# lemerleau/RAFFT

Hardware: AMD Instinct MI355X
Metric: sequences/sec (whole node) on benchmark set, beam N=100; kcal/mol MAE vs CPU (higher is better)
Workload: dtype f32 FFT -> exact int counts, f64 scores, i32 dcal energies

## Files before the change

### rafft_amd/csrc/rafft_config.h

```cpp
#pragma once
#include <cstdio>
#include <cstdlib>
#include <cstring>

struct Config {
    double reserve_frac = 0.10;
    double est = 0.0;
    long linger_us = 600;
    long spin_us = 200, nap_us = 50;
    double big_wave_frac = 0.10;
    int cls1_p = 512;
    int c3_direct = 1;
    int c3_switch = -1;
    int direct_n = 1024;
    int force_fft = 0;
    int prod = 1;
    int no_memo = 0;
    int small_n4 = 16, small_n5 = 32;
    int small_wg = 4;
    int slab = 64;
    int fetch = 4, taper = 25;
    int mat_tile = 64;
    int rl_cap = -1;
    int wide_below = 600;
    int merge_below = -1;
    int merge2_below = -1;
    int split = -1;
    int serial = 0;
    int trace = 0;
    int spans = -1;
    int max_waves = 3;
    int merge_seqs = 16384;
    int trace_alloc = 0;
    int test_hard_fail = -1;
    int test_max_prod = 0;
    int test_ovf_at = -1;
    int seen_fixed = 0;
    int test_cand_limit = 0;
    int seen_bm_max = -1;
    int pad_ = 0;
};
static_assert(sizeof(Config) == 8 * 6 + 4 * 32, "Config: 8-byte fields first, an even number of ints - no padding (same_config compares bytes)");

inline Config read_config()
{
    Config c;
    auto I = [](const char *name, int &v) { if (const char *e = getenv(name)) v = atoi(e); };
    auto L = [](const char *name, long &v) { if (const char *e = getenv(name)) v = atol(e); };
    auto F = [](const char *name, double &v) { if (const char *e = getenv(name)) v = atof(e); };
    auto B = [](const char *name, int &v) { if (getenv(name)) v = 1; };
    I("RAFFT_CLS1_P", c.cls1_p); I("RAFFT_C3_DIRECT", c.c3_direct); I("RAFFT_C3_SWITCH", c.c3_switch); I("RAFFT_DIRECT_N", c.direct_n);
    I("RAFFT_FORCE_FFT", c.force_fft); I("RAFFT_PROD", c.prod); I("RAFFT_NO_MEMO", c.no_memo);
    if (const char *e = getenv("RAFFT_SMALL")) { int a = 16, b = 32; if (sscanf(e, "%d,%d", &a, &b) >= 1) { c.small_n4 = a; c.small_n5 = b; } }
    I("RAFFT_SMALL_WG", c.small_wg); I("RAFFT_SLAB", c.slab); I("RAFFT_FETCH", c.fetch); I("RAFFT_TAPER", c.taper);
    I("RAFFT_WIDE_BELOW", c.wide_below); I("RAFFT_MERGE_BELOW", c.merge_below); I("RAFFT_MERGE2_BELOW", c.merge2_below);
    F("RAFFT_RESERVE_FRAC", c.reserve_frac); I("RAFFT_SPLIT", c.split); I("RAFFT_SERIAL", c.serial);
    I("RAFFT_TRACE", c.trace); if (getenv("RAFFT_TRACE") && c.trace < 1) c.trace = 1;
    I("RAFFT_SPANS", c.spans);
    I("RAFFT_MAX_WAVES", c.max_waves); I("RAFFT_MERGE_SEQS", c.merge_seqs);
    L("RAFFT_LINGER_US", c.linger_us); L("RAFFT_SCHED_SPIN_US", c.spin_us); L("RAFFT_SCHED_NAP_US", c.nap_us); F("RAFFT_BIG_WAVE_FRAC", c.big_wave_frac);
    B("RAFFT_TRACE_ALLOC", c.trace_alloc);
#ifndef RAFFT_NO_TEST_HOOKS
    I("RAFFT_MAT_TILE", c.mat_tile); I("RAFFT_RL_CAP", c.rl_cap); F("RAFFT_EST", c.est); I("RAFFT_SEEN_FIXED", c.seen_fixed);
    I("RAFFT_TEST_CAND_LIMIT", c.test_cand_limit); I("RAFFT_TEST_HARD_FAIL", c.test_hard_fail); I("RAFFT_TEST_MAX_PROD", c.test_max_prod); I("RAFFT_TEST_OVF_AT", c.test_ovf_at);
    I("RAFFT_SEEN_BM_MAX", c.seen_bm_max);
#endif
    return c;
}
inline bool same_config(const Config &a, const Config &b) { return memcmp(&a, &b, sizeof(Config)) == 0; }
```

### rafft_amd/csrc/rafft_kernels.h

```cpp
#pragma once
#include "rafft_device.h"

struct alignas(16) Cand {
    int32_t ddcal;
    uint16_t mi, mj, nb, cut_hi;
    uint32_t cut_lo;
    uint64_t h1, h2;
    __host__ __device__ void set_cuts(int lo0, int hi0, int loo, int hio)
    {
        const unsigned long long v = (unsigned long long)lo0 | ((unsigned long long)hi0 << 12) | ((unsigned long long)loo << 24) | ((unsigned long long)hio << 36);
        cut_lo = (uint32_t)v; cut_hi = (uint16_t)(v >> 32);
    }
    __host__ __device__ void get_cuts(int &lo0, int &hi0, int &loo, int &hio) const
    {
        const unsigned long long v = (unsigned long long)cut_lo | ((unsigned long long)cut_hi << 32);
        lo0 = (int)(v & 4095); hi0 = (int)((v >> 12) & 4095); loo = (int)((v >> 24) & 4095); hio = (int)((v >> 36) & 4095);
    }
};
static_assert(sizeof(Cand) == 32, "Cand must be 32 bytes");

#define NSHARD 64
#ifndef SEEN0
#define SEEN0 8192
#endif
// ... 8 lines not shown
    uint64_t h1, h2;
    uint64_t sp, cursor, combo, total, prod;
    uint64_t c0h1, c0h2;
    uint64_t pad2[3];
};
static_assert(sizeof(StRec) == 128, "StRec is two cache lines");

struct alignas(64) NodeRec {
    int32_t seq, pdcal, n, ci, cj, nbr, ncand, L;
    uint64_t pos, br, cand, soff;
};
static_assert(sizeof(NodeRec) == 64, "NodeRec must be one cache line");

struct ProdEnt { uint32_t cnt; int32_t node; uint64_t off; };
struct alignas(16) MatRec { int32_t sid, sq, L, dcal, nprod, pad; uint64_t combo, prod, soff; };

struct Counters {
    unsigned int n_mat;
    unsigned int overflow;
    unsigned int n_done;
    unsigned int max_nprod;
    unsigned int pad0_[12];
    unsigned long long n_struct, pad1_[7];
    unsigned long long trec_n, tsid_top, pad2_[6];
    unsigned long long seen_top, pad3_[7];
    struct WorkCtr { unsigned int v; unsigned int pad[15]; } n_work[NCLS];
    unsigned long long n_expand, sum_n, sum_lags, n_children, sum_struct_len, n_alias, sum_nbr;
    unsigned long long cls_items[NCLS], cls_sum_n[NCLS], cls_sum_lags[NCLS];
    ShardCtr node[NSHARD], pos[NSHARD], br[NSHARD], sp[NSHARD], cand[NSHARD], node_prev[NSHARD], prod[NSHARD];
    ShardCtr nlist[NSHARD];
    ShardCtr wcur[NCLS][NSHARD];
    unsigned long long wdone[NCLS];
    unsigned long long wdone_pad[8 - NCLS];
    struct StatLine { unsigned long long items, n, lags, nbr, alias, children, struct_len, evals, guessed, kept_guessed, pad[6]; } xstat[NCLS][NSHARD];
};

enum { OVF_STRUCT = 1, OVF_NODE = 2, OVF_POS = 4, OVF_SP = 8, OVF_CAND = 16, OVF_SEEN = 32,
       OVF_TRAJ = 64, OVF_WORK = 128, OVF_PROD = 256, OVF_SORT = 512, OVF_BR = 1024, OVF_LOOPTAB = 2048, OVF_PRODLIST = 4096 };

struct DebugOut {
    int *n_ranked, *lag, *nb, *mi, *mj, *ddcal, *kept;
    double *corval, *score;
};

struct Dev {
    const EnergyTables *T;
    const float2 *tw;
    int S;
    const uint8_t *codes;
    const int *seq_off, *seq_len;
    int K, B, max_branch, min_hp, traj, memo, force_fft, rl_cap, mat_tile, merge_cls;
    double *big_keyv; size_t big_stride;
    int max_prod;
    int fetch_bulk, taper_pct;
    int direct_n;
    int sm_n4, sm_n5;
    int cand_slab;
    int cls1_P, cls1_br;
    int c3_switch;
    double min_nrj, gc, au, gu;
    int *beam, *beam_n, *done, *nsteps;
    int ch_cap;
    uint16_t *ch_parent; uint64_t *ch_combo; int *ch_dcal; uint64_t *ch_h;
    uint64_t *seen; uint64_t seen_cap_total;
    uint64_t *seen_off; uint32_t *seen_cap, *seen_cnt;
    uint32_t *seen_bm;
    uint32_t *seen_mode;
// ... 101 lines not shown
```

### rafft_amd/csrc/rafft_materialize.hip

```cpp
#pragma once


struct MatDesc {
    unsigned long long srcpos, srcbr, cidx;
    int pn, mi, mj, nb, n, nbr, ci, cj, lo0, hi0, loo, hio, a0, b0, ao, bo, flags, win;
    uint32_t newbr;
    int nnod, npos_in, npos_out, nbr_in, nbr_out;
};
__device__ inline MatDesc mat_describe(const Dev &d, int pn, unsigned long long cidx)
{
    MatDesc m;
    m.pn = pn;
    const Cand cd = d.cand[cidx];
    const uint4 *hp = (const uint4 *)&d.nd[pn];
    const uint4 hq0 = hp[0], hq1 = hp[1], hq2 = hp[2];
    m.n = (int)hq0.z; m.ci = (int)hq0.w; m.cj = (int)hq1.x; m.nbr = (int)hq1.y;
    m.srcpos = (unsigned long long)hq2.x | ((unsigned long long)hq2.y << 32); m.srcbr = (unsigned long long)hq2.z | ((unsigned long long)hq2.w << 32);
    m.cidx = cidx;
    m.mi = cd.mi; m.mj = cd.mj; m.nb = cd.nb;
    const uint16_t *pp = d.pos + m.srcpos;
    const int pm = d.pos_packed ? 0x0FFF : 0xFFFF;
    const uint32_t rao = pp[m.mi - m.nb + 1], rbo = pp[m.mj + m.nb - 1];
    m.a0 = pp[m.mi] & pm; m.b0 = pp[m.mj] & pm; m.ao = (int)rao & pm; m.bo = (int)rbo & pm;
    m.newbr = rao | (rbo << 16);
// ... 16 lines not shown
        uint32_t v[U];
#pragma unroll
        for (int u = 0; u < U; u++) {
            const int f = f0 + u * STR;
            v[u] = 0;
            if (f < tp) {
                int lo = 0, hi = 2 * kt - 1;
                while (lo < hi) { const int mid = (lo + hi + 1) >> 1; if (ps[mid] <= f) lo = mid; else hi = mid - 1; }
                const int kk = kb + (lo >> 1), off = f - ps[lo];
                const uint16_t *pp = d.pos + k_srcpos[kk];
                int src;
                if (!(lo & 1)) src = k_mi[kk] + 1 + off;
                else { const int left = k_mi[kk] - k_nb[kk] + 1; src = off < left ? off : k_mj[kk] + k_nb[kk] + (off - left); }
                v[u] = pp[src];
            }
        }
#pragma unroll
        for (int u = 0; u < U; u++) { const int f = f0 + u * STR; if (f < tp) d.pos[pdst + f] = (uint16_t)v[u]; }
    }
    for (int f0 = l; f0 < tbr; f0 += STR * U) {
        uint32_t v[U];
#pragma unroll
        for (int u = 0; u < U; u++) {
            const int f = f0 + u * STR;
            v[u] = 0;
            if (f < tbr) {
                int lo = 0, hi = 2 * kt - 1;
                while (lo < hi) { const int mid = (lo + hi + 1) >> 1; if (bs[mid] <= f) lo = mid; else hi = mid - 1; }
                const int kk = kb + (lo >> 1), off = f - bs[lo];
                const uint32_t *bb = d.br + k_srcbr[kk];
                if (!(lo & 1)) v[u] = bb[k_lo0[kk] + off];
                else {
                    const int loo = k_loo[kk];
                    v[u] = off < loo ? bb[off] : off == loo ? (uint32_t)k_newbr[kk] : bb[k_hio[kk] + (off - loo - 1)];
                }
            }
        }
#pragma unroll
        for (int u = 0; u < U; u++) { const int f = f0 + u * STR; if (f < tbr) d.br[bdst + f] = v[u]; }
    }
    for (int f0 = l; f0 < ts; f0 += STR * U) {
        uint32_t va[U], vb[U];
#pragma unroll
        for (int u = 0; u < U; u++) {
            const int f = f0 + u * STR;
            va[u] = 0; vb[u] = 0;
            if (f < ts) {
                int lo = 0, hi = kt - 1;
                while (lo < hi) { const int mid = (lo + hi + 1) >> 1; if (ns[mid] <= f) lo = mid; else hi = mid - 1; }
                const int t = f - ns[lo];
                const uint16_t *pp = d.pos + k_srcpos[kb + lo];
                va[u] = pp[k_mi[kb + lo] - t]; vb[u] = pp[k_mj[kb + lo] + t];
            }
        }
#pragma unroll
        for (int u = 0; u < U; u++) { const int f = f0 + u * STR; if (f < ts) d.sp[sdst + f] = (uint32_t)(va[u] & pmask) | ((uint32_t)(vb[u] & pmask) << 16); }
    }
}

#ifndef RAFFT_MAT_WAVES
#define RAFFT_MAT_WAVES 1
#endif
constexpr int MAT_NT = 64;
constexpr int MAT4_TL = 16;
constexpr int MAT4_TEAMS = 64 / MAT4_TL;
constexpr int MAT4_PROD = 64;

template <int TL>
__device__ __forceinline__ int team_incl_scan(int x, int tl)
{
    if constexpr (TL == 16) return row16_incl_scan(x);
    else {
        static_assert(TL == 64, "a team is one DPP row or the whole wavefront");
        for (int o = 1; o < 64; o <<= 1) { const int y = __shfl_up(x, o, 64); if (tl >= o) x += y; }
        return x;
    }
}
template <int TL>
__device__ __forceinline__ int team_sum(int x)
{
    if constexpr (TL == 16) return __shfl(row16_incl_scan(x), TL - 1, TL);
    else {
        for (int o = 32; o > 0; o >>= 1) x += __shfl_xor(x, o, 64);
        return x;
    }
}

template <int TL>
__device__ __forceinline__ void materialize_body(const Dev d, int n_mat, unsigned long long *prod_off, int *prod_node, int *prod_cnt,
                                                 int *sel, int cap)
{
    constexpr int TEAMS = 64 / TL;
    const int tid = threadIdx.x, team = tid / TL, tl = tid % TL;
    __shared__ unsigned long long k_srcpos[64], k_srcbr[64];
    __shared__ int k_mi[64], k_mj[64], k_nb[64], k_lo0[64], k_loo[64], k_hio[64], k_newbr[64];
    __shared__ int ps_[TEAMS][2 * TL + 1], bs_[TEAMS][2 * TL + 1], ns_[TEAMS][TL + 1];
    __shared__ unsigned long long sh64_[TEAMS][5];
    int *ps = ps_[team], *bs = bs_[team], *ns = ns_[team];
    const int tb = team * TL;
    const unsigned long long tmask = (~0ULL >> (64 - TL)) << tb;
    if (d.c->overflow) return;
    for (int mat_i0 = blockIdx.x * TEAMS; mat_i0 < n_mat; mat_i0 += gridDim.x * TEAMS) {
    const int mat_i = mat_i0 + team;
    const bool live = mat_i < n_mat;
    MatRec rec;
    rec.sid = 0; rec.sq = 0; rec.L = 0; rec.dcal = 0; rec.nprod = 0; rec.combo = 0; rec.prod = 0; rec.soff = 0;
    if (live) rec = d.mat[mat_i];
    const int sid = rec.sid, sq = rec.sq, L = rec.L, my_dcal = rec.dcal;
    const uint64_t soff = rec.soff;
    const int pmask = d.pos_packed ? 0x0FFF : 0xFFFF;
    int mprod = rec.nprod;
    if (mprod > cap) mprod = cap;
    {
        const ProdEnt *pl = d.prod + rec.prod;
        for (int k = tl; k < mprod; k += TL) { const ProdEnt pe = pl[k]; prod_node[k] = pe.node; prod_cnt[k] = (int)pe.cnt; prod_off[k] = pe.off; sel[k] = 0; }
    }
    wave_sync();
    if (tl == 0) {
        unsigned long long idx = rec.combo;
        for (int k = mprod - 1; k >= 0 && idx; k--) {
            const unsigned int c = (unsigned int)prod_cnt[k];
            if (idx < (1ULL << 24)) {
                const unsigned int v = (unsigned int)idx;
                unsigned int q = (unsigned int)((float)v * __frcp_rn((float)c));
                int r = (int)(v - q * c);
                if (r < 0) { q--; r += (int)c; } else if (r >= (int)c) { q++; r -= (int)c; }
                sel[k] = r; idx = q;
            } else { const unsigned long long q = idx / c; sel[k] = (int)(idx - q * c); idx = q; }
        }
    }
    wave_sync();

    const int TILE = d.mat_tile < TL ? d.mat_tile : TL;
    const bool one_tile = mprod <= TILE;
    const bool memo = d.memo != 0;
    MatDesc md;
    md.flags = 0; md.win = 0; md.nnod = 0; md.npos_in = md.npos_out = md.nbr_in = md.nbr_out = 0; md.nb = 0; md.cidx = 0;
    int tot_nodes = 0, tot_new = 0, tot_pos = 0, tot_br = 0, tot_sp = 0;
    for (int base = 0; base < mprod; base += TILE) {
        const int k = base + tl;
        int nnod = 0, nnew = 0, npos = 0, nbrr = 0, nsp = 0;
        if (k < mprod && tl < TILE) {
            const unsigned long long cidx = prod_off[k] + (unsigned long long)sel[k];
            unsigned long long old = 0;
            if (memo) old = atomicOr(&d.cslot[cidx], 0x8000000080000000ULL);
            md = mat_describe(d, prod_node[k], cidx);
            int win = md.flags;
            if (memo) win &= ((old >> 31) & 1ULL ? 0 : 1) | ((old >> 63) & 1ULL ? 0 : 2);
            md.win = win;
            if (!one_tile) sel[k] |= win << 28;
            nnod = md.nnod; nnew = (win & 1) + (win >> 1); nsp = md.nb;
            npos = ((win & 1) ? md.npos_in : 0) + ((win & 2) ? md.npos_out : 0);
            nbrr = ((win & 1) ? md.nbr_in : 0) + ((win & 2) ? md.nbr_out : 0);
        }
        nnod = team_sum<TL>(nnod); nnew = team_sum<TL>(nnew); npos = team_sum<TL>(npos); nbrr = team_sum<TL>(nbrr); nsp = team_sum<TL>(nsp);
        tot_nodes += nnod; tot_new += nnew; tot_pos += npos; tot_br += nbrr; tot_sp += nsp;
    }
    bool ok = live;
    if (tl < 5 && live) {
        const int shd = mat_i & (NSHARD - 1);
        unsigned long long *ctr = tl == 0 ? &d.c->node[shd].v : tl == 1 ? &d.c->pos[shd].v : tl == 2 ? &d.c->sp[shd].v : tl == 3 ? &d.c->br[shd].v : &d.c->nlist[shd].v;
        const unsigned long long want = tl == 0 ? (unsigned long long)tot_new : tl == 1 ? (unsigned long long)tot_pos
                                      : tl == 2 ? (unsigned long long)tot_sp : tl == 3 ? (unsigned long long)tot_br : (unsigned long long)tot_nodes;
        const unsigned long long cap = tl == 0 || tl == 4 ? d.nd_shard_cap : tl == 1 ? d.pos_shard_cap : tl == 2 ? d.sp_shard_cap : d.br_shard_cap;
        const unsigned long long b0 = want ? atomicAdd(ctr, want) : 0ULL;
        const bool bad = b0 + want > cap;
        if (bad) atomicOr(&d.c->overflow, tl == 0 || tl == 4 ? OVF_NODE : tl == 1 ? OVF_POS : tl == 2 ? OVF_SP : OVF_BR);
        const unsigned long long origin = tl == 0 || tl == 4 ? d.nd_base : tl == 1 ? d.pos_base : 0ULL;
        sh64_[team][tl] = origin + (unsigned long long)shd * cap + b0;
        ok = !bad;
    }
    ok = ((__ballot(!ok) & tmask) == 0ULL) && live;
    wave_sync();
    if (!ok) { if (tl == 0 && live) { d.st[sid].nnodes = 0; d.st[sid].node0 = 0; d.st[sid].sp = 0; d.st[sid].nsp = 0; } }
    const unsigned long long nbase = sh64_[team][0], pbase = sh64_[team][1], sbase = sh64_[team][2], bbase = sh64_[team][3], lbase = sh64_[team][4];

    int run_nodes = 0, run_new = 0, run_pos = 0, run_br = 0, run_sp = 0;
    const int mp2 = ok ? mprod : 0;
    for (int base = 0; base < mp2; base += TILE) {
        const int k = base + tl;
        const int kt = mp2 - base < TILE ? mp2 - base : TILE;
        if (!one_tile) {
            md.flags = 0; md.win = 0; md.nnod = 0; md.npos_in = md.npos_out = md.nbr_in = md.nbr_out = 0; md.nb = 0;
            if (k < mp2 && tl < TILE) { md = mat_describe(d, prod_node[k], prod_off[k] + (unsigned long long)(sel[k] & 0x0FFFFFFF)); md.win = (sel[k] >> 28) & 3; }
        }
        const bool act = k < mp2 && tl < TILE;
        const int cp_in = act && (md.win & 1) ? md.npos_in : 0, cp_out = act && (md.win & 2) ? md.npos_out : 0;
        const int cb_in = act && (md.win & 1) ? md.nbr_in : 0, cb_out = act && (md.win & 2) ? md.nbr_out : 0;
        int xn = act ? md.nnod : 0, xw = act ? (md.win & 1) + (md.win >> 1) : 0, xp = cp_in + cp_out, xb = cb_in + cb_out, xs = act ? md.nb : 0;
        const int vn = xn, vw = xw, vp = xp, vb = xb, vs = xs;
        xn = team_incl_scan<TL>(xn, tl); xw = team_incl_scan<TL>(xw, tl); xp = team_incl_scan<TL>(xp, tl); xb = team_incl_scan<TL>(xb, tl);
        xs = team_incl_scan<TL>(xs, tl);
        const int tn = __shfl(xn, TL - 1, TL), tw = __shfl(xw, TL - 1, TL), tp = __shfl(xp, TL - 1, TL), tbr = __shfl(xb, TL - 1, TL),
                  ts = __shfl(xs, TL - 1, TL);
        const int p0 = xp - vp, b0 = xb - vb;
        ps[2 * tl] = p0; ps[2 * tl + 1] = p0 + cp_in;
        bs[2 * tl] = b0; bs[2 * tl + 1] = b0 + cb_in;
        ns[tl] = xs - vs;
        if (tl == 0) { ps[2 * TL] = tp; bs[2 * TL] = tbr; ns[TL] = ts; }
        if (act) {
            k_srcpos[tid] = md.srcpos; k_srcbr[tid] = md.srcbr;
            k_mi[tid] = md.mi; k_mj[tid] = md.mj; k_nb[tid] = md.nb; k_lo0[tid] = md.lo0; k_loo[tid] = md.loo; k_hio[tid] = md.hio;
            k_newbr[tid] = (int)md.newbr;
            int nid = (int)(nbase + run_new + (xw - vw));
            unsigned long long le = lbase + run_nodes + (xn - vn);
            const unsigned long long poff = pbase + run_pos + p0, boff = bbase + run_br + b0;
            const int slot0 = (int)(2 * md.cidx);
            if (md.flags & 1) {
                if (md.win & 1) {
                    d.nd[nid].seq = sq; d.nd[nid].pdcal = my_dcal; d.nd[nid].pos = poff; d.nd[nid].n = md.npos_in;
                    d.nd[nid].L = L; d.nd[nid].soff = soff;
                    d.nd[nid].ci = md.a0; d.nd[nid].cj = md.b0; d.nd[nid].br = boff; d.nd[nid].nbr = md.nbr_in;
                    d.nd[nid].ncand = -1; d.nd[nid].cand = 0;
                    if (memo) { d.nd_slot[nid] = (uint32_t)slot0; ((uint32_t *)d.cslot)[slot0] = (uint32_t)(nid + 1) | 0x80000000u; }
                    d.nlist[le] = memo ? -(slot0 + 1) : nid;
                    nid++;
                } else d.nlist[le] = -(slot0 + 1);
                le++;
            }
            if (md.flags & 2) {
                if (md.win & 2) {
                    d.nd[nid].seq = sq; d.nd[nid].pdcal = my_dcal; d.nd[nid].pos = poff + cp_in; d.nd[nid].n = md.npos_out;
                    d.nd[nid].L = L; d.nd[nid].soff = soff;
                    d.nd[nid].ci = md.ci; d.nd[nid].cj = md.cj; d.nd[nid].br = boff + cb_in; d.nd[nid].nbr = md.nbr_out;
                    d.nd[nid].ncand = -1; d.nd[nid].cand = 0;
                    if (memo) { d.nd_slot[nid] = (uint32_t)(slot0 + 1); ((uint32_t *)d.cslot)[slot0 + 1] = (uint32_t)(nid + 1) | 0x80000000u; }
                    d.nlist[le] = memo ? -(slot0 + 2) : nid;
                } else d.nlist[le] = -(slot0 + 2);
            }
        }
        wave_sync();
        mat_copy_tile<TL, 4>(d, tl, tb, kt, ps, bs, ns, k_srcpos, k_srcbr, k_mi, k_mj, k_nb, k_lo0, k_loo, k_hio, k_newbr, tp, tbr, ts,
                             pbase + run_pos, bbase + run_br, sbase + run_sp, pmask);
        run_nodes += tn; run_new += tw; run_pos += tp; run_br += tbr; run_sp += ts;
        wave_sync();
    }
    if (ok && tl == 0) { d.st[sid].node0 = (int)lbase; d.st[sid].nnodes = tot_nodes; d.st[sid].sp = sbase; d.st[sid].nsp = tot_sp; }
    wave_sync();
    }
}

__global__ __launch_bounds__(MAT_NT, RAFFT_MAT_WAVES) void materialize_kernel(Dev d, int n_mat)
{
    extern __shared__ __align__(16) uint8_t mat_dyn[];
    unsigned long long *prod_off = (unsigned long long *)mat_dyn;
    int *prod_node = (int *)(prod_off + d.max_prod);
    int *prod_cnt = prod_node + d.max_prod;
    int *sel = prod_cnt + d.max_prod;
    materialize_body<MAT_NT>(d, n_mat, prod_off, prod_node, prod_cnt, sel, d.max_prod);
}

__global__ __launch_bounds__(64, RAFFT_MAT_WAVES) void materialize_team_kernel(Dev d, int n_mat)
{
    __shared__ unsigned long long prod_off_[MAT4_TEAMS][MAT4_PROD];
    __shared__ int prod_node_[MAT4_TEAMS][MAT4_PROD], prod_cnt_[MAT4_TEAMS][MAT4_PROD], sel_[MAT4_TEAMS][MAT4_PROD];
    const int team = threadIdx.x / MAT4_TL;
    materialize_body<MAT4_TL>(d, n_mat, prod_off_[team], prod_node_[team], prod_cnt_[team], sel_[team], MAT4_PROD);
}


struct NodeWords { uint4 q0, q1, q2; };
__device__ __forceinline__ NodeWords load_node_words(const Dev &d, int nid)
{
    const uint4 *hp = (const uint4 *)&d.nd[nid];
    NodeWords w;
    w.q0 = hp[0]; w.q1 = hp[1]; w.q2 = hp[2];
    pin(w.q0); pin(w.q1); pin(w.q2);
    return w;
}
__device__ inline bool same_loop(const Dev &d, const NodeWords &a, int b)
{
    const NodeWords o = load_node_words(d, b);
    if (a.q0.x != o.q0.x || a.q0.z != o.q0.z || a.q0.w != o.q0.w || a.q1.x != o.q1.x || a.q1.y != o.q1.y) return false;
    const uint32_t *x = d.br + ((unsigned long long)a.q2.z | ((unsigned long long)a.q2.w << 32));
    const uint32_t *y = d.br + ((unsigned long long)o.q2.z | ((unsigned long long)o.q2.w << 32));
    const int k = (int)a.q1.y;
    for (int i = 0; i < k; i += 4) {
        unsigned int xa[4], ya[4];
#pragma unroll
        for (int u = 0; u < 4; u++) { xa[u] = i + u < k ? x[i + u] : 0u; ya[u] = i + u < k ? y[i + u] : 0u; }
#pragma unroll
        for (int u = 0; u < 4; u++) { pin(xa[u]); pin(ya[u]); }
        if (xa[0] != ya[0] || xa[1] != ya[1] || xa[2] != ya[2] || xa[3] != ya[3]) return false;
    }
    return true;
}

#ifndef DEDUPE_NT
#define DEDUPE_NT 512
#endif
// ... 88 lines not shown
```

### rafft_amd/csrc/rafft_wave.h

```cpp
#pragma once

namespace {

hipEvent_t next_event(std::vector<hipEvent_t> &used)
{
    hipEvent_t e = nullptr;
    if (!g.ev_free.empty()) { e = g.ev_free.back(); g.ev_free.pop_back(); }
    else if (hipEventCreate(&e) != hipSuccess) return nullptr;
    used.push_back(e);
    return e;
}

struct Span { hipEvent_t a, b; int kind; };
static int g_span_level = 1;
static inline bool span_on(int kind) { return g_span_level >= 2 || (g_span_level == 1 && kind == 11); }
#define SPAN_REC(ev, st, kind) do { if (span_on(kind)) HIPCHK(hipEventRecord((ev), (st))); } while (0)

struct HostOut {
    std::vector<rafft_seq_result> seq;
    std::vector<std::vector<int>> step_size, step_off;
    std::vector<int> one_size, one_off;
    std::vector<const char *> db_ptr;
    std::vector<const int *> dcal_ptr;
    std::vector<std::shared_ptr<struct PinChunk>> chunks;
// ... 338 lines not shown
        }
        if (int rc = launch_expand_cls(cfg, d, cls, cf, grid, cs)) return rc;
        if (cls == 1) bt.stats.n_expand_launches++;
        SPAN_REC(sp.b, cs, sp.kind);
        spans.push_back(sp);
        if (!inline_) {
            HIPCHK(hipEventRecord(ws.ev_join[cls], cs));
            HIPCHK(hipStreamWaitEvent(st, ws.ev_join[cls], 0));
        }
    }
    SPAN_REC(wall.b, st, 4);
    spans.push_back(wall);
    {
        Span sp{next_event(), next_event(), 1};
        SPAN_REC(sp.a, st, sp.kind);
        if (n_active < wide_below) hipLaunchKernelGGL((beam_step_kernel<1024>), dim3((unsigned)S), dim3(1024), bs_lds[1], st, d, c.sort_cap, (int)bs_bm[1]);
        else hipLaunchKernelGGL((beam_step_kernel<256>), dim3((unsigned)S), dim3(256), bs_lds[0], st, d, c.sort_cap, (int)bs_bm[0]);
        HIPCHK(hipGetLastError());
        SPAN_REC(sp.b, st, sp.kind);
        spans.push_back(sp);
    }
    steps++;
    HIPCHK(hipMemcpyAsync(ws.hot, ws.counters.p, hot_len, hipMemcpyDeviceToHost, st));
    HIPCHK(hipEventRecord(ws.ev_hot, st));
    t_issued = std::chrono::steady_clock::now();
    return 0;
}

int Wave::issue_materialize(unsigned nm)
{
    hipStream_t st = ws.stream;
    Span sp{next_event(), next_event(), 2};
    SPAN_REC(sp.a, st, sp.kind);
    if (d.max_prod <= MAT4_PROD)
        hipLaunchKernelGGL(materialize_team_kernel, dim3((nm + MAT4_TEAMS - 1) / MAT4_TEAMS), dim3(64), 0, st, d, (int)nm);
    else hipLaunchKernelGGL(materialize_kernel, dim3(nm), dim3(MAT_NT), mat_lds, st, d, (int)nm);
    HIPCHK(hipGetLastError());
    const unsigned merge_below = cfg.merge_below >= 0 ? (unsigned)cfg.merge_below : 2u * (unsigned)g.n_cu;
    const unsigned merge2_below = cfg.merge2_below >= 0 ? (unsigned)cfg.merge2_below : 128u * (unsigned)g.n_cu;
    d.merge_cls = seam ? 0 : nm < merge_below ? merge_target : nm < merge2_below ? 2 : 0;
    merged_now = d.merge_cls;
    const unsigned dd_grid = std::min<unsigned>((unsigned)g.n_cu * (1024u / DEDUPE_NT), (unsigned)std::min<unsigned long long>(0x7fffffffULL, (unsigned long long)nm * 4ULL / DEDUPE_NT + 2ULL));
    hipLaunchKernelGGL(dedupe_kernel, dim3(dd_grid), dim3(DEDUPE_NT), 0, st, d);
    HIPCHK(hipGetLastError());
    SPAN_REC(sp.b, st, sp.kind);
    spans.push_back(sp);
    return 0;
}

int Wave::after_beam()
{
    HostTimer acc_{ms_after};
    hipStream_t st = ws.stream;
    if (draining) return finish_done();
    const size_t hot_len = offsetof(Counters, node);
    memcpy(&hc, ws.hot, hot_len);
    if (hc.overflow) { ovf = hc.overflow; return finish(); }
    if (cfg.test_ovf_at >= 0 && depth == 0 && steps == cfg.test_ovf_at) { ovf = OVF_STRUCT; return finish(); }
    if (hc.n_mat == 0) return finish();
    n_active = (unsigned)S - hc.n_done;
    last_mat = hc.n_mat;
    const bool harvest_now = !p.traj && !seam && !harvested && S >= 256 && (size_t)hc.trec_n * 10 >= S * 7;
    const size_t harvest_n = (size_t)hc.trec_n;
    if (int rc = issue_materialize(hc.n_mat)) return rc;
    if (cfg.trace >= 2) {
        Counters h2;
        HIPCHK(hipMemcpyAsync(&h2, ws.counters.p, hot_len, hipMemcpyDeviceToHost, st));
        HIPCHK(hipStreamSynchronize(st));
        fprintf(stderr, "[rafft] step %d: n_mat %u -> work %u %u %u %u | small %u %u\n", steps, hc.n_mat, h2.n_work[0].v, h2.n_work[1].v, h2.n_work[2].v, h2.n_work[3].v, h2.n_work[4].v, h2.n_work[5].v);
// ... 126 lines not shown
            const double sh = hc.n_expand ? (double)hc.cls_items[c] / (double)hc.n_expand : 0.0;
            const int64_t v = 3 * (int64_t)hc.cls_sum_n[c] + 16 * (int64_t)hc.cls_sum_lags[c] + (int64_t)(sh * 3.0 * (double)(hc.sum_struct_len + sumL));
            if (c == 2) bt.stats.alg_bytes_expand_c2 += v;
            else if (c == 3 || c == 0) bt.stats.alg_bytes_expand_c3 += v;
            else if (c >= NGEN) bt.stats.alg_bytes_expand_small += v;
        }
        bt.stats.alg_bytes_beam += 2 * (int64_t)hc.sum_struct_len + 8 * (int64_t)(hc.n_struct - S);
        bt.stats.alg_bytes_expand_all += ex;
        bt.stats.alg_bytes += ex + 2 * (int64_t)hc.sum_struct_len + 8 * (int64_t)(hc.n_struct - S);
    }


    tail.stats = since(tail.t0);
    if (int rc = emit_rows(harvested, (size_t)hc.trec_n - harvested, false, &tail.gather)) return rc;
    tail.gather += tail.stats;
    if (harvested) {
        HIPCHK(hipEventRecord(ws.ev_copy, ws.copy_stream));
        HIPCHK(hipStreamWaitEvent(st, ws.ev_copy, 0));
    }
    HIPCHK(hipEventRecord(ws.ev_hot, st));
    finished = false; draining = true;
    return 0;
}

int Wave::finish_done_body()
{
    finished = true;
    const double tl_copy = since(tail.t0);
    const long long tot_bytes = last_rows_bytes;
    if (cfg.trace) {
        auto mx = [&](const ShardCtr *sc) { unsigned long long m = 0, t = 0; for (int i = 0; i < NSHARD; i++) { m = std::max(m, sc[i].v); t += sc[i].v; } return std::make_pair(m, t); };
        auto nd = mx(hc.node), po = mx(hc.pos), br = mx(hc.br), spr = mx(hc.sp), ca = mx(hc.cand), pr = mx(hc.prod), nl = mx(hc.nlist);
        fprintf(stderr, "[rafft] max productive regions per structure: %u (limit %d)\n", hc.max_nprod, d.max_prod);
        fprintf(stderr, "[rafft] arenas used/cap (max shard | total): st %llu/%zu  nd %llu/%llu|%llu  pos %llu/%llu|%llu  br %llu/%llu|%llu  sp %llu/%llu|%llu  cand %llu/%llu|%llu  prod %llu/%llu|%llu  nlist %llu/%llu|%llu  seen %llu/%zu  est %.1f\n",
                hc.n_struct, c.st, nd.first, (unsigned long long)d.nd_shard_cap, nd.second, po.first, (unsigned long long)d.pos_shard_cap, po.second,
                br.first, (unsigned long long)d.br_shard_cap, br.second, spr.first, (unsigned long long)d.sp_shard_cap, spr.second,
                ca.first, (unsigned long long)d.cand_shard_cap, ca.second, pr.first, (unsigned long long)d.prod_shard_cap, pr.second, nl.first, (unsigned long long)d.nd_shard_cap, nl.second, hc.seen_top, c.seen, est);
    }
    if (cfg.trace >= 2) {
        std::vector<uint32_t> cnt(S), cap(S);
        HIPCHK(hipMemcpy(cnt.data(), d.seen_cnt, S * 4, hipMemcpyDeviceToHost));
        HIPCHK(hipMemcpy(cap.data(), d.seen_cap, S * 4, hipMemcpyDeviceToHost));
        const int edges[] = {0, 80, 100, 130, 200, 300, 500, 1000, 2000, 1 << 30};
        for (int e = 0; e + 1 < (int)(sizeof(edges) / sizeof(edges[0])); e++) {
            unsigned long long n = 0, sum = 0, mxc = 0, grown = 0, slots = 0;
            for (size_t i = 0; i < S; i++) if (len[i] > edges[e] && len[i] <= edges[e + 1]) { n++; sum += cnt[i]; mxc = std::max<unsigned long long>(mxc, cnt[i]); grown += cap[i] > seen_cap0[i] ? 1 : 0; slots += cap[i]; }
            if (n) fprintf(stderr, "[rafft] seen sets, %d < L <= %d: %llu sequences, mean %llu entries, max %llu, %llu grew, %llu slots at the end\n", edges[e], edges[e + 1], n, sum / n, mxc, grown, slots);
        }
    }
    if (cfg.trace) fprintf(stderr, "[rafft] host time inside issue_step %.3f ms, inside after_beam (incl. nested issue_step and this tail) %.3f ms\n", ms_issue, ms_after);
    if (cfg.trace) fprintf(stderr, "[rafft] wave S=%zu setup %.2f ms, loop %.2f ms (%d steps), tail %.2f ms (counters %.3f, records+gather %.3f, rows out %.3f incl. %.1f MB D2H)\n",
                                       S, ms_setup, tail.ms_loop, steps, since(tail.t0), tail.stats, tail.gather - tail.stats, tl_copy - tail.gather, (double)tot_bytes / 1e6);
    return result = 0;
}

int run_seam(Batch &bt, const std::vector<SeqIn> &one, const SeamIn &sm)
{
    Wave w(g.ws[0], {std::shared_ptr<Batch>(&bt, [](Batch *) {})}, one, 4.0, &sm);
    if (int rc = w.setup()) return rc;
    Workspace &W = g.ws[0];
    {
        std::vector<uint16_t> packed(sm.pos);
        if (w.d.pos_packed) {
            for (auto &v : packed) v = (uint16_t)(v | (kBaseCode[(unsigned char)one[0].s[v]] << 12));
        }
        HIPCHK(hipMemcpy(W.pos.p, packed.data(), packed.size() * 2, hipMemcpyHostToDevice));
// ... 27 lines not shown
```

Before: 550,900.

## Compute combo digits per lane in team materialize and drop LDS product lists

The team materialize kernel no longer stages the product lists (node, count, offset) in shared memory. Each lane keeps its own product entry in registers and works out its combo digit with a saturating suffix-product scan across the team, which replaces the serial digit loop on lane 0. The kernel becomes a template over team size, with an optional 8-lane team chosen by a new config knob, and the one-tile path reuses the descriptor from the first pass instead of calling mat_describe again. It also adds per-shard counters for materialized structures and multi-tile cases, printed under trace. These counters cost an extra atomic per block, and the scan adds 64-bit multiplies and divides per lane.

```diff
diff --git a/rafft_amd/csrc/rafft_config.h b/rafft_amd/csrc/rafft_config.h
--- a/rafft_amd/csrc/rafft_config.h
+++ b/rafft_amd/csrc/rafft_config.h
@@ -38,7 +38,7 @@
     int seen_fixed = 0;
     int test_cand_limit = 0;
     int seen_bm_max = -1;
-    int pad_ = 0;
+    int mat_team = 16;
 };
 static_assert(sizeof(Config) == 8 * 6 + 4 * 32, "Config: 8-byte fields first, an even number of ints - no padding (same_config compares bytes)");
 
@@ -61,7 +61,7 @@
     L("RAFFT_LINGER_US", c.linger_us); L("RAFFT_SCHED_SPIN_US", c.spin_us); L("RAFFT_SCHED_NAP_US", c.nap_us); F("RAFFT_BIG_WAVE_FRAC", c.big_wave_frac);
     B("RAFFT_TRACE_ALLOC", c.trace_alloc);
 #ifndef RAFFT_NO_TEST_HOOKS
-    I("RAFFT_MAT_TILE", c.mat_tile); I("RAFFT_RL_CAP", c.rl_cap); F("RAFFT_EST", c.est); I("RAFFT_SEEN_FIXED", c.seen_fixed);
+    I("RAFFT_MAT_TILE", c.mat_tile); I("RAFFT_MAT_TEAM", c.mat_team); I("RAFFT_RL_CAP", c.rl_cap); F("RAFFT_EST", c.est); I("RAFFT_SEEN_FIXED", c.seen_fixed);
     I("RAFFT_TEST_CAND_LIMIT", c.test_cand_limit); I("RAFFT_TEST_HARD_FAIL", c.test_hard_fail); I("RAFFT_TEST_MAX_PROD", c.test_max_prod); I("RAFFT_TEST_OVF_AT", c.test_ovf_at);
     I("RAFFT_SEEN_BM_MAX", c.seen_bm_max);
 #endif
diff --git a/rafft_amd/csrc/rafft_kernels.h b/rafft_amd/csrc/rafft_kernels.h
--- a/rafft_amd/csrc/rafft_kernels.h
+++ b/rafft_amd/csrc/rafft_kernels.h
@@ -64,7 +64,7 @@
     ShardCtr wcur[NCLS][NSHARD];
     unsigned long long wdone[NCLS];
     unsigned long long wdone_pad[8 - NCLS];
-    struct StatLine { unsigned long long items, n, lags, nbr, alias, children, struct_len, evals, guessed, kept_guessed, pad[6]; } xstat[NCLS][NSHARD];
+    struct StatLine { unsigned long long items, n, lags, nbr, alias, children, struct_len, evals, guessed, kept_guessed, mat, mat_tiles, pad[4]; } xstat[NCLS][NSHARD];
 };
 
 enum { OVF_STRUCT = 1, OVF_NODE = 2, OVF_POS = 4, OVF_SP = 8, OVF_CAND = 16, OVF_SEEN = 32,
diff --git a/rafft_amd/csrc/rafft_materialize.hip b/rafft_amd/csrc/rafft_materialize.hip
--- a/rafft_amd/csrc/rafft_materialize.hip
+++ b/rafft_amd/csrc/rafft_materialize.hip
@@ -72,7 +72,8 @@
                 if (!(lo & 1)) v[u] = bb[k_lo0[kk] + off];
                 else {
                     const int loo = k_loo[kk];
-                    v[u] = off < loo ? bb[off] : off == loo ? (uint32_t)k_newbr[kk] : bb[k_hio[kk] + (off - loo - 1)];
+                    v[u] = (uint32_t)k_newbr[kk];
+                    if (off != loo) v[u] = bb[off < loo ? off : k_hio[kk] + (off - loo - 1)];
                 }
             }
         }
@@ -102,46 +103,93 @@
 #define RAFFT_MAT_WAVES 1
 #endif
 constexpr int MAT_NT = 64;
-constexpr int MAT4_TL = 16;
-constexpr int MAT4_TEAMS = 64 / MAT4_TL;
 constexpr int MAT4_PROD = 64;
 
 template <int TL>
 __device__ __forceinline__ int team_incl_scan(int x, int tl)
 {
     if constexpr (TL == 16) return row16_incl_scan(x);
-    else {
-        static_assert(TL == 64, "a team is one DPP row or the whole wavefront");
+    else if constexpr (TL == 8) {
+        const int y1 = __builtin_amdgcn_update_dpp(0, x, 0x111, 0xF, 0xF, true);
+        x += tl >= 1 ? y1 : 0;
+        const int y2 = __builtin_amdgcn_update_dpp(0, x, 0x112, 0xF, 0xF, true);
+        x += tl >= 2 ? y2 : 0;
+        x += __builtin_amdgcn_update_dpp(0, x, 0x114, 0xF, 0xA, true);
+        return x;
+    } else {
+        static_assert(TL == 64, "a team is half a DPP row, one row or the whole wavefront");
         for (int o = 1; o < 64; o <<= 1) { const int y = __shfl_up(x, o, 64); if (tl >= o) x += y; }
         return x;
     }
 }
 template <int TL>
-__device__ __forceinline__ int team_sum(int x)
-{
-    if constexpr (TL == 16) return __shfl(row16_incl_scan(x), TL - 1, TL);
+__device__ __forceinline__ int team_sum(int x, int tl)
+{
+    if constexpr (TL < 64) return __shfl(team_incl_scan<TL>(x, tl), TL - 1, TL);
     else {
         for (int o = 32; o > 0; o >>= 1) x += __shfl_xor(x, o, 64);
         return x;
     }
 }
 
+__device__ __forceinline__ unsigned long long combo_divmod(unsigned long long idx, unsigned int c, unsigned int &rem)
+{
+    if (idx < (1ULL << 24)) {
+        const unsigned int v = (unsigned int)idx;
+        unsigned int q = (unsigned int)((float)v * __frcp_rn((float)c));
+        int r = (int)(v - q * c);
+        if (r < 0) { q--; r += (int)c; } else if (r >= (int)c) { q++; r -= (int)c; }
+        rem = (unsigned int)r;
+        return q;
+    }
+    const unsigned long long q = idx / c;
+    rem = (unsigned int)(idx - q * c);
+    return q;
+}
+__device__ __forceinline__ void combo_digits_serial(unsigned long long idx, const int *cnt, int *sel, int mprod)
+{
+    for (int k = mprod - 1; k >= 0; k--) {
+        unsigned int r = 0;
+        if (idx) idx = combo_divmod(idx, (unsigned int)cnt[k], r);
+        sel[k] = (int)r;
+    }
+}
 template <int TL>
+__device__ __forceinline__ int combo_digit_lanes(unsigned long long idx, unsigned int cnt, int tl)
+{
+    const unsigned long long sat = idx + 1;
+    unsigned long long s = cnt < sat ? cnt : sat;
+#pragma unroll
+    for (int o = 1; o < TL; o <<= 1) {
+        const unsigned long long y = __shfl_down(s, o, TL);
+        if (tl + o < TL) { const unsigned long long lo = s * y; s = (__umul64hi(s, y) || lo > sat) ? sat : lo; }
+    }
+    s = __shfl_down(s, 1, TL);
+    if (tl == TL - 1) s = 1;
+    if (s > idx) return 0;
+    unsigned int r;
+    const unsigned long long q = s < (1ULL << 24) && idx < (1ULL << 24)
+        ? (unsigned long long)combo_divmod(idx, (unsigned int)s, r) : idx / s;
+    combo_divmod(q, cnt, r);
+    return (int)r;
+}
+
+template <int TL, bool LISTS>
 __device__ __forceinline__ void materialize_body(const Dev d, int n_mat, unsigned long long *prod_off, int *prod_node, int *prod_cnt,
                                                  int *sel, int cap)
 {
     constexpr int TEAMS = 64 / TL;
+    static_assert(TL >= 5, "five lanes of a team allocate from the five arenas");
     const int tid = threadIdx.x, team = tid / TL, tl = tid % TL;
     __shared__ unsigned long long k_srcpos[64], k_srcbr[64];
     __shared__ int k_mi[64], k_mj[64], k_nb[64], k_lo0[64], k_loo[64], k_hio[64], k_newbr[64];
     __shared__ int ps_[TEAMS][2 * TL + 1], bs_[TEAMS][2 * TL + 1], ns_[TEAMS][TL + 1];
     __shared__ unsigned long long sh64_[TEAMS][5];
-    int *ps = ps_[team], *bs = bs_[team], *ns = ns_[team];
     const int tb = team * TL;
-    const unsigned long long tmask = (~0ULL >> (64 - TL)) << tb;
     if (d.c->overflow) return;
-    for (int mat_i0 = blockIdx.x * TEAMS; mat_i0 < n_mat; mat_i0 += gridDim.x * TEAMS) {
-    const int mat_i = mat_i0 + team;
+    unsigned int st_mat = 0, st_tiles = 0;
+    {
+    const int mat_i = blockIdx.x * TEAMS + team;
     const bool live = mat_i < n_mat;
     MatRec rec;
     rec.sid = 0; rec.sq = 0; rec.L = 0; rec.dcal = 0; rec.nprod = 0; rec.combo = 0; rec.prod = 0; rec.soff = 0;
@@ -151,28 +199,36 @@
     const int pmask = d.pos_packed ? 0x0FFF : 0xFFFF;
     int mprod = rec.nprod;
     if (mprod > cap) mprod = cap;
-    {
-        const ProdEnt *pl = d.prod + rec.prod;
-        for (int k = tl; k < mprod; k += TL) { const ProdEnt pe = pl[k]; prod_node[k] = pe.node; prod_cnt[k] = (int)pe.cnt; prod_off[k] = pe.off; sel[k] = 0; }
-    }
-    wave_sync();
-    if (tl == 0) {
-        unsigned long long idx = rec.combo;
-        for (int k = mprod - 1; k >= 0 && idx; k--) {
-            const unsigned int c = (unsigned int)prod_cnt[k];
-            if (idx < (1ULL << 24)) {
-                const unsigned int v = (unsigned int)idx;
-                unsigned int q = (unsigned int)((float)v * __frcp_rn((float)c));
-                int r = (int)(v - q * c);
-                if (r < 0) { q--; r += (int)c; } else if (r >= (int)c) { q++; r -= (int)c; }
-                sel[k] = r; idx = q;
-            } else { const unsigned long long q = idx / c; sel[k] = (int)(idx - q * c); idx = q; }
-        }
-    }
-    wave_sync();
-
     const int TILE = d.mat_tile < TL ? d.mat_tile : TL;
     const bool one_tile = mprod <= TILE;
+    if (tl == 0 && live) { st_mat++; st_tiles += one_tile ? 0 : 1; }
+    const ProdEnt *pl = d.prod + rec.prod;
+    int my_node = 0, my_sel = 0;
+    unsigned long long my_off = 0;
+    if constexpr (LISTS) {
+        for (int k = tl; k < mprod; k += TL) { const ProdEnt pe = pl[k]; prod_node[k] = pe.node; prod_cnt[k] = (int)pe.cnt; prod_off[k] = pe.off; }
+        wave_sync();
+        if (tl == 0) combo_digits_serial(rec.combo, prod_cnt, sel, mprod);
+        wave_sync();
+    } else {
+        unsigned int cnt = 1;
+        if (one_tile && tl < mprod) { const ProdEnt pe = pl[tl]; my_node = pe.node; my_off = pe.off; cnt = pe.cnt; }
+        my_sel = combo_digit_lanes<TL>(rec.combo, cnt, tl);
+        if (!one_tile) for (int k = tl; k < mprod; k += TL) sel[k] = (int)pl[k].cnt;
+        wave_sync();
+        if (!one_tile && tl == 0) combo_digits_serial(rec.combo, sel, sel, mprod);
+        wave_sync();
+    }
+    auto entry = [&](int k, int &node) -> unsigned long long {
+        if constexpr (LISTS) { node = prod_node[k]; return prod_off[k] + (unsigned long long)(sel[k] & 0x0FFFFFFF); }
+        else {
+            if (one_tile) { node = my_node; return my_off + (unsigned long long)my_sel; }
+            const ProdEnt pe = pl[k];
+            node = pe.node;
+            return pe.off + (unsigned long long)(sel[k] & 0x0FFFFFFF);
+        }
+    };
+
     const bool memo = d.memo != 0;
     MatDesc md;
     md.flags = 0; md.win = 0; md.nnod = 0; md.npos_in = md.npos_out = md.nbr_in = md.nbr_out = 0; md.nb = 0; md.cidx = 0;
@@ -181,10 +237,11 @@
         const int k = base + tl;
         int nnod = 0, nnew = 0, npos = 0, nbrr = 0, nsp = 0;
         if (k < mprod && tl < TILE) {
-            const unsigned long long cidx = prod_off[k] + (unsigned long long)sel[k];
+            int node;
+            const unsigned long long cidx = entry(k, node);
             unsigned long long old = 0;
             if (memo) old = atomicOr(&d.cslot[cidx], 0x8000000080000000ULL);
-            md = mat_describe(d, prod_node[k], cidx);
+            md = mat_describe(d, node, cidx);
             int win = md.flags;
             if (memo) win &= ((old >> 31) & 1ULL ? 0 : 1) | ((old >> 63) & 1ULL ? 0 : 2);
             md.win = win;
@@ -193,7 +250,7 @@
             npos = ((win & 1) ? md.npos_in : 0) + ((win & 2) ? md.npos_out : 0);
             nbrr = ((win & 1) ? md.nbr_in : 0) + ((win & 2) ? md.nbr_out : 0);
         }
-        nnod = team_sum<TL>(nnod); nnew = team_sum<TL>(nnew); npos = team_sum<TL>(npos); nbrr = team_sum<TL>(nbrr); nsp = team_sum<TL>(nsp);
+        nnod = team_sum<TL>(nnod, tl); nnew = team_sum<TL>(nnew, tl); npos = team_sum<TL>(npos, tl); nbrr = team_sum<TL>(nbrr, tl); nsp = team_sum<TL>(nsp, tl);
         tot_nodes += nnod; tot_new += nnew; tot_pos += npos; tot_br += nbrr; tot_sp += nsp;
     }
     bool ok = live;
@@ -210,24 +267,24 @@
         sh64_[team][tl] = origin + (unsigned long long)shd * cap + b0;
         ok = !bad;
     }
-    ok = ((__ballot(!ok) & tmask) == 0ULL) && live;
+    ok = ((__ballot(!ok) & ((~0ULL >> (64 - TL)) << tb)) == 0ULL) && live;
     wave_sync();
-    if (!ok) { if (tl == 0 && live) { d.st[sid].nnodes = 0; d.st[sid].node0 = 0; d.st[sid].sp = 0; d.st[sid].nsp = 0; } }
-    const unsigned long long nbase = sh64_[team][0], pbase = sh64_[team][1], sbase = sh64_[team][2], bbase = sh64_[team][3], lbase = sh64_[team][4];
+    if (tl == 0 && live) {
+        if (ok) { d.st[sid].node0 = (int)sh64_[team][4]; d.st[sid].nnodes = tot_nodes; d.st[sid].sp = sh64_[team][2]; d.st[sid].nsp = tot_sp; }
+        else { d.st[sid].nnodes = 0; d.st[sid].node0 = 0; d.st[sid].sp = 0; d.st[sid].nsp = 0; }
+    }
 
     int run_nodes = 0, run_new = 0, run_pos = 0, run_br = 0, run_sp = 0;
     const int mp2 = ok ? mprod : 0;
-    for (int base = 0; base < mp2; base += TILE) {
+    auto tile2 = [&](const MatDesc &m, int base) __attribute__((always_inline)) {
+        int *ps = ps_[team], *bs = bs_[team], *ns = ns_[team];
+        const unsigned long long *ab = sh64_[team];
         const int k = base + tl;
         const int kt = mp2 - base < TILE ? mp2 - base : TILE;
-        if (!one_tile) {
-            md.flags = 0; md.win = 0; md.nnod = 0; md.npos_in = md.npos_out = md.nbr_in = md.nbr_out = 0; md.nb = 0;
-            if (k < mp2 && tl < TILE) { md = mat_describe(d, prod_node[k], prod_off[k] + (unsigned long long)(sel[k] & 0x0FFFFFFF)); md.win = (sel[k] >> 28) & 3; }
-        }
         const bool act = k < mp2 && tl < TILE;
-        const int cp_in = act && (md.win & 1) ? md.npos_in : 0, cp_out = act && (md.win & 2) ? md.npos_out : 0;
-        const int cb_in = act && (md.win & 1) ? md.nbr_in : 0, cb_out = act && (md.win & 2) ? md.nbr_out : 0;
-        int xn = act ? md.nnod : 0, xw = act ? (md.win & 1) + (md.win >> 1) : 0, xp = cp_in + cp_out, xb = cb_in + cb_out, xs = act ? md.nb : 0;
+        const int cp_in = act && (m.win & 1) ? m.npos_in : 0, cp_out = act && (m.win & 2) ? m.npos_out : 0;
+        const int cb_in = act && (m.win & 1) ? m.nbr_in : 0, cb_out = act && (m.win & 2) ? m.nbr_out : 0;
+        int xn = act ? m.nnod : 0, xw = act ? (m.win & 1) + (m.win >> 1) : 0, xp = cp_in + cp_out, xb = cb_in + cb_out, xs = act ? m.nb : 0;
         const int vn = xn, vw = xw, vp = xp, vb = xb, vs = xs;
         xn = team_incl_scan<TL>(xn, tl); xw = team_incl_scan<TL>(xw, tl); xp = team_incl_scan<TL>(xp, tl); xb = team_incl_scan<TL>(xb, tl);
         xs = team_incl_scan<TL>(xs, tl);
@@ -239,18 +296,18 @@
         ns[tl] = xs - vs;
         if (tl == 0) { ps[2 * TL] = tp; bs[2 * TL] = tbr; ns[TL] = ts; }
         if (act) {
-            k_srcpos[tid] = md.srcpos; k_srcbr[tid] = md.srcbr;
-            k_mi[tid] = md.mi; k_mj[tid] = md.mj; k_nb[tid] = md.nb; k_lo0[tid] = md.lo0; k_loo[tid] = md.loo; k_hio[tid] = md.hio;
-            k_newbr[tid] = (int)md.newbr;
-            int nid = (int)(nbase + run_new + (xw - vw));
-            unsigned long long le = lbase + run_nodes + (xn - vn);
-            const unsigned long long poff = pbase + run_pos + p0, boff = bbase + run_br + b0;
-            const int slot0 = (int)(2 * md.cidx);
-            if (md.flags & 1) {
-                if (md.win & 1) {
-                    d.nd[nid].seq = sq; d.nd[nid].pdcal = my_dcal; d.nd[nid].pos = poff; d.nd[nid].n = md.npos_in;
+            k_srcpos[tid] = m.srcpos; k_srcbr[tid] = m.srcbr;
+            k_mi[tid] = m.mi; k_mj[tid] = m.mj; k_nb[tid] = m.nb; k_lo0[tid] = m.lo0; k_loo[tid] = m.loo; k_hio[tid] = m.hio;
+            k_newbr[tid] = (int)m.newbr;
+            int nid = (int)(ab[0] + run_new + (xw - vw));
+            unsigned long long le = ab[4] + run_nodes + (xn - vn);
+            const unsigned long long poff = ab[1] + run_pos + p0, boff = ab[3] + run_br + b0;
+            const int slot0 = (int)(2 * m.cidx);
+            if (m.flags & 1) {
+                if (m.win & 1) {
+                    d.nd[nid].seq = sq; d.nd[nid].pdcal = my_dcal; d.nd[nid].pos = poff; d.nd[nid].n = m.npos_in;
                     d.nd[nid].L = L; d.nd[nid].soff = soff;
-                    d.nd[nid].ci = md.a0; d.nd[nid].cj = md.b0; d.nd[nid].br = boff; d.nd[nid].nbr = md.nbr_in;
+                    d.nd[nid].ci = m.a0; d.nd[nid].cj = m.b0; d.nd[nid].br = boff; d.nd[nid].nbr = m.nbr_in;
                     d.nd[nid].ncand = -1; d.nd[nid].cand = 0;
                     if (memo) { d.nd_slot[nid] = (uint32_t)slot0; ((uint32_t *)d.cslot)[slot0] = (uint32_t)(nid + 1) | 0x80000000u; }
                     d.nlist[le] = memo ? -(slot0 + 1) : nid;
@@ -258,11 +315,11 @@
                 } else d.nlist[le] = -(slot0 + 1);
                 le++;
             }
-            if (md.flags & 2) {
-                if (md.win & 2) {
-                    d.nd[nid].seq = sq; d.nd[nid].pdcal = my_dcal; d.nd[nid].pos = poff + cp_in; d.nd[nid].n = md.npos_out;
+            if (m.flags & 2) {
+                if (m.win & 2) {
+                    d.nd[nid].seq = sq; d.nd[nid].pdcal = my_dcal; d.nd[nid].pos = poff + cp_in; d.nd[nid].n = m.npos_out;
                     d.nd[nid].L = L; d.nd[nid].soff = soff;
-                    d.nd[nid].ci = md.ci; d.nd[nid].cj = md.cj; d.nd[nid].br = boff + cb_in; d.nd[nid].nbr = md.nbr_out;
+                    d.nd[nid].ci = m.ci; d.nd[nid].cj = m.cj; d.nd[nid].br = boff + cb_in; d.nd[nid].nbr = m.nbr_out;
                     d.nd[nid].ncand = -1; d.nd[nid].cand = 0;
                     if (memo) { d.nd_slot[nid] = (uint32_t)(slot0 + 1); ((uint32_t *)d.cslot)[slot0 + 1] = (uint32_t)(nid + 1) | 0x80000000u; }
                     d.nlist[le] = memo ? -(slot0 + 2) : nid;
@@ -271,12 +328,25 @@
         }
         wave_sync();
         mat_copy_tile<TL, 4>(d, tl, tb, kt, ps, bs, ns, k_srcpos, k_srcbr, k_mi, k_mj, k_nb, k_lo0, k_loo, k_hio, k_newbr, tp, tbr, ts,
-                             pbase + run_pos, bbase + run_br, sbase + run_sp, pmask);
+                             ab[1] + run_pos, ab[3] + run_br, ab[2] + run_sp, pmask);
         run_nodes += tn; run_new += tw; run_pos += tp; run_br += tbr; run_sp += ts;
         wave_sync();
-    }
-    if (ok && tl == 0) { d.st[sid].node0 = (int)lbase; d.st[sid].nnodes = tot_nodes; d.st[sid].sp = sbase; d.st[sid].nsp = tot_sp; }
+    };
+    if (one_tile) { if (mp2 > 0) tile2(md, 0); }
+    else for (int base = 0; base < mp2; base += TILE) {
+        const int k = base + tl;
+        MatDesc m;
+        m.flags = 0; m.win = 0; m.nnod = 0; m.npos_in = m.npos_out = m.nbr_in = m.nbr_out = 0; m.nb = 0; m.cidx = 0;
+        if (k < mp2 && tl < TILE) { int node; const unsigned long long cidx = entry(k, node); m = mat_describe(d, node, cidx); m.win = (sel[k] >> 28) & 3; }
+        tile2(m, base);
+    }
     wave_sync();
+    }
+    for (int o = 32; o >= TL; o >>= 1) { st_mat += __shfl_xor(st_mat, o, 64); st_tiles += __shfl_xor(st_tiles, o, 64); }
+    if (tid == 0) {
+        Counters::StatLine &x = d.c->xstat[0][blockIdx.x & (NSHARD - 1)];
+        if (st_mat) atomicAdd(&x.mat, (unsigned long long)st_mat);
+        if (st_tiles) atomicAdd(&x.mat_tiles, (unsigned long long)st_tiles);
     }
 }
 
@@ -287,15 +357,14 @@
     int *prod_node = (int *)(prod_off + d.max_prod);
     int *prod_cnt = prod_node + d.max_prod;
     int *sel = prod_cnt + d.max_prod;
-    materialize_body<MAT_NT>(d, n_mat, prod_off, prod_node, prod_cnt, sel, d.max_prod);
-}
-
+    materialize_body<MAT_NT, true>(d, n_mat, prod_off, prod_node, prod_cnt, sel, d.max_prod);
+}
+
+template <int TL>
 __global__ __launch_bounds__(64, RAFFT_MAT_WAVES) void materialize_team_kernel(Dev d, int n_mat)
 {
-    __shared__ unsigned long long prod_off_[MAT4_TEAMS][MAT4_PROD];
-    __shared__ int prod_node_[MAT4_TEAMS][MAT4_PROD], prod_cnt_[MAT4_TEAMS][MAT4_PROD], sel_[MAT4_TEAMS][MAT4_PROD];
-    const int team = threadIdx.x / MAT4_TL;
-    materialize_body<MAT4_TL>(d, n_mat, prod_off_[team], prod_node_[team], prod_cnt_[team], sel_[team], MAT4_PROD);
+    __shared__ int sel_[64 / TL][MAT4_PROD];
+    materialize_body<TL, false>(d, n_mat, nullptr, nullptr, nullptr, sel_[threadIdx.x / TL], MAT4_PROD);
 }
 
 
diff --git a/rafft_amd/csrc/rafft_wave.h b/rafft_amd/csrc/rafft_wave.h
--- a/rafft_amd/csrc/rafft_wave.h
+++ b/rafft_amd/csrc/rafft_wave.h
@@ -394,9 +394,10 @@
     hipStream_t st = ws.stream;
     Span sp{next_event(), next_event(), 2};
     SPAN_REC(sp.a, st, sp.kind);
-    if (d.max_prod <= MAT4_PROD)
-        hipLaunchKernelGGL(materialize_team_kernel, dim3((nm + MAT4_TEAMS - 1) / MAT4_TEAMS), dim3(64), 0, st, d, (int)nm);
-    else hipLaunchKernelGGL(materialize_kernel, dim3(nm), dim3(MAT_NT), mat_lds, st, d, (int)nm);
+    if (d.max_prod <= MAT4_PROD) {
+        if (cfg.mat_team == 8) hipLaunchKernelGGL(materialize_team_kernel<8>, dim3((nm + 7) / 8), dim3(64), 0, st, d, (int)nm);
+        else hipLaunchKernelGGL(materialize_team_kernel<16>, dim3((nm + 3) / 4), dim3(64), 0, st, d, (int)nm);
+    } else hipLaunchKernelGGL(materialize_kernel, dim3(nm), dim3(MAT_NT), mat_lds, st, d, (int)nm);
     HIPCHK(hipGetLastError());
     const unsigned merge_below = cfg.merge_below >= 0 ? (unsigned)cfg.merge_below : 2u * (unsigned)g.n_cu;
     const unsigned merge2_below = cfg.merge2_below >= 0 ? (unsigned)cfg.merge2_below : 128u * (unsigned)g.n_cu;
@@ -589,6 +590,9 @@
         auto mx = [&](const ShardCtr *sc) { unsigned long long m = 0, t = 0; for (int i = 0; i < NSHARD; i++) { m = std::max(m, sc[i].v); t += sc[i].v; } return std::make_pair(m, t); };
         auto nd = mx(hc.node), po = mx(hc.pos), br = mx(hc.br), spr = mx(hc.sp), ca = mx(hc.cand), pr = mx(hc.prod), nl = mx(hc.nlist);
         fprintf(stderr, "[rafft] max productive regions per structure: %u (limit %d)\n", hc.max_nprod, d.max_prod);
+        unsigned long long n_mat = 0, n_tiles = 0;
+        for (int i = 0; i < NSHARD; i++) { n_mat += hc.xstat[0][i].mat; n_tiles += hc.xstat[0][i].mat_tiles; }
+        fprintf(stderr, "[rafft] materialize: %llu structures, %llu in more than one tile\n", n_mat, n_tiles);
         fprintf(stderr, "[rafft] arenas used/cap (max shard | total): st %llu/%zu  nd %llu/%llu|%llu  pos %llu/%llu|%llu  br %llu/%llu|%llu  sp %llu/%llu|%llu  cand %llu/%llu|%llu  prod %llu/%llu|%llu  nlist %llu/%llu|%llu  seen %llu/%zu  est %.1f\n",
                 hc.n_struct, c.st, nd.first, (unsigned long long)d.nd_shard_cap, nd.second, po.first, (unsigned long long)d.pos_shard_cap, po.second,
                 br.first, (unsigned long long)d.br_shard_cap, br.second, spr.first, (unsigned long long)d.sp_shard_cap, spr.second,
```

New measurement: 549,400, median of 2. Within noise of the previous version (-0.3%).
